# upb-lea/gym-electric-motor

Measured on AMD Instinct MI355X. Metric: env-steps/sec (batched PMSM, tau=1e-4), higher is better.
Workload: dtype f32; 1 GPU; Finite-CC-PMSM-v0 (Finite-B6C + dq transform), RK4, fp32, tau=1e-4, default constraint + auto-reset; 16384 envs/GPU x 1 GPU(s); one bench step = one fused launch of 1000 control steps, obs [K,N,S_out] rows + done bytes written for every control step; env_id=Finite-CC-PMSM-v0, envs_per_gpu=16384, solver=rk4, steps_per_launch=1000, parallelism=env-sharded x1, no data-path collective, world_size=1, oversubscribed=False

## Files before the change

### gym_electric_motor_amd/csrc/gemx_capi.hip

```cpp
#include <dlfcn.h>

#include <cstdarg>
#include <cstdio>
#include <cstdlib>
#include <cstring>
#include <mutex>
#include <new>
#include <set>
#include <string>

#include "gemx_common.hpp"

namespace gemx {

template <class R>
__device__ void reset_obs_row(int sys, const DevParams<R> &P, const double *y, double eps, int nd, int nout, double *o) {
    const double us = (double)P.u_sup, s3 = sqrt(3.0);
    for (int j = 0; j < nout; ++j) o[j] = 0.0;
    const double ua = -0.5 * us, ual = 2.0 / 3.0 * (ua - 0.5 * ua - 0.5 * ua), ube = 2.0 / 3.0 * (0.5 * s3 * ua - 0.5 * s3 * ua);
    if (eps > kPi) eps -= kTwoPi;
    if (sys == GEMX_SYS_SYNC || sys == GEMX_SYS_EESM) {
        const double c = cos(eps), s = sin(eps);
        const double al = c * y[1] - s * y[2], be = s * y[1] + c * y[2];
        o[0] = y[0];
// ... 593 lines not shown

    int ndev = 0;
    if (hipGetDeviceCount(&ndev) != hipSuccess || ndev <= 0) {
        delete h;
        return fail(GEMX_ERR_DEVICE, "no HIP device visible: the gemx stepper has no CPU fallback");
    }
    if (device < 0 || device >= ndev) { delete h; return fail(GEMX_ERR_ARG, "device %d out of range (0..%d)", device, ndev - 1); }
    gemx::DeviceGuard guard(device);
    {
        gemx_unit_launch_fn fn = nullptr;
        rc = load_unit(cfg->system_kind, h->conv_unit, cfg->dtype == GEMX_F64 ? 1 : 0, &fn);
        if (rc != GEMX_OK) { delete h; return rc; }
        h->unit_launch = (void *)fn;
    }
    {
        int cur = -1;
        if (hipGetDevice(&cur) != hipSuccess || cur != device) { delete h; return fail(GEMX_ERR_DEVICE, "hipSetDevice(%d) failed", device); }
        hipDeviceProp_t prop;
        if (hipGetDeviceProperties(&prop, device) == hipSuccess) {
            if (prop.multiProcessorCount > 0) h->n_cu = prop.multiProcessorCount;
            if (prop.sharedMemPerBlock >= 64 * 1024) h->lds_max = prop.sharedMemPerBlock;
            if (strncmp(prop.gcnArchName, "gfx950", 6) != 0 || prop.multiProcessorCount != 256) h->pace_gbps = 0.0;
        }
        for (const char *name : {"GEMX_STEPS_PER_BLOCK", "GEMX_PIPE", "GEMX_PIPE_SHAPE", "GEMX_STEP_KERNEL", "GEMX_DC_STREAM", "GEMX_DCS_EPW", "GEMX_LINMAP", "GEMX_PACE_GBPS", "GEMX_PACE_CAL"}) {
            const char *v = getenv(name);
            if (v == nullptr) continue;
            const size_t used = strlen(h->overrides);
            snprintf(h->overrides + used, sizeof(h->overrides) - used, "%s%s=%.16s", used ? " " : "", name, v);
        }
        const char *ev = getenv("GEMX_STEPS_PER_BLOCK");
        if (ev) h->steps_per_block = atoi(ev);
        ev = getenv("GEMX_PIPE");
        if (ev) h->use_pipe = atoi(ev);
        ev = getenv("GEMX_PIPE_SHAPE");
        if (ev) h->pipe_shape = atoi(ev);
        ev = getenv("GEMX_STEP_KERNEL");
        if (ev) h->use_step_kernel = atoi(ev);
        ev = getenv("GEMX_DC_STREAM");
        if (ev) h->use_dc_stream = atoi(ev);
        ev = getenv("GEMX_DCS_EPW");
        if (ev) h->dcs_epw = atoi(ev);
        ev = getenv("GEMX_PACE_GBPS");
        if (ev) h->pace_gbps = atof(ev);
        ev = getenv("GEMX_PACE_CAL");
        if (ev) h->pace_cal_on = atoi(ev);
        ev = getenv("GEMX_LINMAP");
        if (ev && atoi(ev) == 0) h->linmap_state = -1;

    }
    host_reset_obs(*h, m);

    const size_t es = (size_t)elem_size(h);
    auto cleanup = [&](int code) { gemx_destroy(h); return code; };
    h->extra_rows = (cfg->solver_flags & GEMX_SOLVER_ADAPTIVE) ? 3 : (cfg->supply_kind == GEMX_SUPPLY_RC ? 2 : 0);
    if (hipMalloc(&h->state, es * (h->nd + h->extra_rows) * (size_t)h->n) != hipSuccess) return cleanup(fail(GEMX_ERR_ALLOC, "hipMalloc(state) failed"));
    if (h->extra_rows && hipMemset((char *)h->state + es * (size_t)h->nd * (size_t)h->n, 0, es * (size_t)h->extra_rows * (size_t)h->n) != hipSuccess)
        return cleanup(fail(GEMX_ERR_DEVICE, "hipMemset failed"));
    if (h->has_angle && hipMalloc(&h->angle, (cfg->dtype == GEMX_F64 ? 8 : 4) * (size_t)h->n) != hipSuccess)
        return cleanup(fail(GEMX_ERR_ALLOC, "hipMalloc(angle) failed"));
    if (hipMalloc((void **)&h->sw, (size_t)h->n * h->sw_rows) != hipSuccess) return cleanup(fail(GEMX_ERR_ALLOC, "hipMalloc(sw) failed"));
    if (cfg->action_delay > 0) {
        const bool disc = c == GEMX_CONV_FINITE_B6 || c == GEMX_CONV_FINITE_4QC || c == GEMX_CONV_FINITE_2X4QC || c == GEMX_CONV_FINITE_B6_4QC ||
                          c == GEMX_CONV_FINITE_2XB6;
        h->ring_bytes = (size_t)cfg->action_delay * (size_t)h->n * (disc ? 1 : (size_t)h->nact_conv * es);
        if (hipMalloc(&h->ring, h->ring_bytes) != hipSuccess) return cleanup(fail(GEMX_ERR_ALLOC, "hipMalloc(delay ring) failed"));
    }
    if (cfg->init_kind != GEMX_INIT_CONST) {
        InitDev I;
        memset(&I, 0, sizeof(I));
        I.kind = cfg->init_kind;
// ... 366 lines not shown
    HIP_TRY(hipMemcpyAsync(out_dev, h->sw, (size_t)h->n * h->sw_rows, hipMemcpyDeviceToDevice, (hipStream_t)stream));
    return GEMX_OK;
}
int gemx_set_switch_state(gemx_handle *h, const uint8_t *in_dev, void *stream) {
    if (!h || !in_dev) return fail(GEMX_ERR_ARG, "null argument");
    gemx::DeviceGuard guard(h->device);
    HIP_TRY(hipMemcpyAsync(h->sw, in_dev, (size_t)h->n * h->sw_rows, hipMemcpyDeviceToDevice, (hipStream_t)stream));
    return GEMX_OK;
}
const char *gemx_last_launch(const gemx_handle *h) {
    if (!h) return "";
    const auto &l = h->ll;
    if (l.pipe == 3)
        snprintf(h->last_launch, sizeof(h->last_launch),
                 "gemx::dc_stream_kernel<sys=%d,conv=%d,solver=%d,f32,D=%d> grid=%lld x %d threads, lds=%zu B, K=%d", l.sys, l.conv, l.solver, l.d,
                 l.blocks, l.threads, l.lds, l.k);
    else if (l.pipe == 2)
        snprintf(h->last_launch, sizeof(h->last_launch), "gemx::step_kernel<sys=%d,conv=%d,load=%d,solver=%d,il=%d,%s> grid=%lld x %d threads, K=1", l.sys, l.conv,
                 l.load, l.solver, l.il, l.real_size == 4 ? "f32" : "f64", l.blocks, l.threads);
    else if (l.pipe) {
        snprintf(h->last_launch, sizeof(h->last_launch),
                 "gemx::advance_pipe_kernel<sys=%d,conv=%d,load=%d,solver=%d,il=%d,%s,D=%d> grid=%lld x %d threads, lds=%zu B, K=%d", l.sys,
                 l.conv, l.load, l.solver, l.il, l.real_size == 4 ? "f32" : "f64", l.d, l.blocks, l.threads, l.lds, l.k);
        if (l.pace != 0) {
            const size_t used = strlen(h->last_launch);
            snprintf(h->last_launch + used, sizeof(h->last_launch) - used, ", rate limit %u0 ns per block (%lld resident workgroups%s)", l.pace,
                     l.pace_res < l.blocks ? l.pace_res : l.blocks, l.pace_tail != 0 ? "; shorter in the last round" : "");
        }
        if (h->pace_cal_state != 0) {
            const size_t used = strlen(h->last_launch);
            snprintf(h->last_launch + used, sizeof(h->last_launch) - used, ", limiter %s at %.2f x the built-in target%s", h->pace_cal_state == 2 ? "calibrated" : "calibrating",
                     h->pace_scale_last, h->pace_scale_last == 0.0 ? " (unpaced)" : "");
        }
    } else
        snprintf(h->last_launch, sizeof(h->last_launch),
                 "gemx::advance_kernel<sys=%d,conv=%d,load=%d,solver=%d,il=%d,%s> grid=%lld x %d threads, lds=%zu B, K=%d, S=%d", l.sys, l.conv,
                 l.load, l.solver, l.il, l.real_size == 4 ? "f32" : "f64", l.blocks, l.threads, l.lds, l.k, l.s);
    if (h->overrides[0] != 0) {
        const size_t used = strlen(h->last_launch);
        snprintf(h->last_launch + used, sizeof(h->last_launch) - used, " overrides[%s]", h->overrides);
    }
    return h->last_launch;
}
int gemx_set_steps_per_block(gemx_handle *h, int32_t steps) {
    if (!h || steps < 0) return fail(GEMX_ERR_ARG, "invalid argument");
    h->steps_per_block = steps;
// ... 12 lines not shown
```

### gym_electric_motor_amd/csrc/gemx_common.hpp

```cpp
#pragma once
#include <hip/hip_runtime.h>

#include <cmath>
#include <cstdint>
#include <cstring>
#include <type_traits>

#include "gemx.h"

namespace gemx {

constexpr int BLOCK = 64;
constexpr double kTwoPi = 6.283185307179586476925286766559;
constexpr double kPi = 3.141592653589793238462643383279;

template <int SYS> struct SysTraits;
template <> struct SysTraits<GEMX_SYS_DC_PERMEX> { static constexpr int ND = 2, NOUT = 5, HAS_ANGLE = 0; };
template <> struct SysTraits<GEMX_SYS_SYNC>      { static constexpr int ND = 3, NOUT = 14, HAS_ANGLE = 1; };
template <> struct SysTraits<GEMX_SYS_SCIM>      { static constexpr int ND = 5, NOUT = 14, HAS_ANGLE = 1; };
template <> struct SysTraits<GEMX_SYS_DC_SERIES> { static constexpr int ND = 2, NOUT = 5, HAS_ANGLE = 0; };
template <> struct SysTraits<GEMX_SYS_DC_SHUNT>  { static constexpr int ND = 3, NOUT = 6, HAS_ANGLE = 0; };
template <> struct SysTraits<GEMX_SYS_DC_EXTEX>  { static constexpr int ND = 3, NOUT = 7, HAS_ANGLE = 0; };
template <> struct SysTraits<GEMX_SYS_EESM>      { static constexpr int ND = 4, NOUT = 16, HAS_ANGLE = 1; };
template <> struct SysTraits<GEMX_SYS_DFIM>      { static constexpr int ND = 5, NOUT = 24, HAS_ANGLE = 1; };
// ... 365 lines not shown
    unsigned char *ring;
    uint32_t *fifo_phase;
    uint32_t *err;
    const InitDev *rinit;
    uint32_t *rcnt;
    const RewardDev<R> *rw;
    const R *refs;
    R *reward;
    int64_t N;
    int32_t K, obs_every;
    int32_t S;
    int32_t D;
    int32_t coop;
    int32_t obs_vec;
    uint32_t pace_block_ticks;
    uint32_t pace_tail_ticks;
    uint32_t pace_tail_from;
    uint64_t act_seed;
    int64_t act_env_base;
    int32_t prep_phases;
    int32_t act_half;
    uint32_t act_step0;
    int32_t act_synth;
};

template <class R> __device__ __forceinline__ int fifo_phase_read(const KArgs<R> &a) {
    return a.P.delay > 0 ? (int)*a.fifo_phase : 0;
}
template <class R> __device__ __forceinline__ void fifo_phase_advance(const KArgs<R> &a, int phase, bool one_lane) {
    if (a.P.delay > 0 && one_lane) {
        const uint32_t ticket = atomicAdd(a.fifo_phase + 1, 1u);
        if (ticket == gridDim.x - 1) {
            a.fifo_phase[1] = 0u;
            a.fifo_phase[0] = (uint32_t)((phase + a.K) % a.P.delay);
        }
    }
}

constexpr int MAX_ACT_CHUNKS = 12;
constexpr int MAX_STEPS_PER_BLOCK = 32;
constexpr int PIPE_D = 12, PIPE_OUT_WAVES = 3;
constexpr int PIPE_D2 = 4, PIPE_OUT_WAVES2 = 2;
constexpr int PIPE_OUT_WAVES_RW = 6;
constexpr int PIPE_D3 = 2, PIPE_OUT_WAVES3 = 2;
constexpr int pipe_loader_waves(int) { return 1; }
constexpr int PIPE_ACT_BUFS = 2;
#ifndef GEMX_PIPE_AHEAD2
#define GEMX_PIPE_AHEAD2 0
#endif
constexpr int pipe_act_ahead(int D) { return (D <= 4 && GEMX_PIPE_AHEAD2) ? 2 : 1; }
constexpr int pipe_act_bufs(int D) { return pipe_act_ahead(D) + 1; }
constexpr int pipe_ref_bufs(int D) { return pipe_act_ahead(D) + 2; }
__host__ __device__ constexpr int pipe_queue_rows(int D, int delay, bool dq_processor, bool full) {
    return (D == PIPE_D && !full && dq_processor && delay > 0) ? D + delay : delay;
}
__host__ __device__ constexpr int act_chunks(int cpr) {
    return (MAX_STEPS_PER_BLOCK * cpr + BLOCK - 1) / BLOCK < MAX_ACT_CHUNKS ? (MAX_STEPS_PER_BLOCK * cpr + BLOCK - 1) / BLOCK : MAX_ACT_CHUNKS;
}

}

struct gemx_handle {
    gemx_config cfg;
    int64_t n;
    int device;
    int nd, nout, nact, has_angle;
// ... 14 lines not shown
    gemx::RewardHot<float> rh_f = {};
    gemx::RewardHot<double> rh_d = {};
    int rw_n_ref = -1;
    bool cur_half = false;
    bool cur_synth = false;
    uint64_t cur_seed = 0;
    uint32_t cur_step0 = 0;
    const void *cur_refs = nullptr;
    void *cur_reward = nullptr;
    void *ring = nullptr;
    size_t ring_bytes = 0;
    int nact_conv = 1;
    int conv_unit = 0;
    void *unit_launch = nullptr;
    unsigned long long steps_total = 0;
    uint32_t *fifo_phase = nullptr;
    uint32_t *err = nullptr;
    void *reset_obs_dev = nullptr;
    void *cw_dev = nullptr;
    double reset_obs[GEMX_MAX_OUT];
    int n_cu = 256;
    size_t lds_max = 160 * 1024;
    int steps_per_block = 0;
    struct LastLaunch { int pipe, sys, conv, load, solver, il, real_size, d, threads, k, s; long long blocks; size_t lds; unsigned pace, pace_tail; long long pace_res; int shape; };
    LastLaunch ll = {};
    mutable char last_launch[512] = "";
    char overrides[192] = "";
    double pace_gbps = -1.0;
    struct PaceCal {
        static constexpr int NC = 5, SAMPLES = 6, RING = 16;
        long long sig = -1;
        float center = 1.0f;
        int recenters = 0;
        static constexpr int MAX_RECENTER = 4;
        int next = 0;
        int chosen = -1;
        float best[NC] = {1e30f, 1e30f, 1e30f, 1e30f, 1e30f};
        int count[NC] = {0, 0, 0, 0, 0};
        int issued[NC] = {0, 0, 0, 0, 0};
        void *ev0[RING] = {}, *ev1[RING] = {};
        int ev_cand[RING];
        bool ev_init = false;
    } pcal;
    int pace_cal_on = 1;
    double pace_scale_last = 1.0;
    int pace_cal_state = 0;
    size_t pipe_occ_smem[8] = {0, 0, 0, 0, 0, 0, 0, 0};
    int pipe_occ[8] = {0, 0, 0, 0, 0, 0, 0, 0};
    int pipe_regs[8] = {0, 0, 0, 0, 0, 0, 0, 0};
// ... 45 lines not shown
```

### gym_electric_motor_amd/csrc/gemx_kernels.hpp

```cpp
#pragma once
#include <cstdio>

#include "gemx_common.hpp"

namespace gemx {

__device__ __forceinline__ float med3_r(float x, float lo, float hi) { return __builtin_amdgcn_fmed3f(x, lo, hi); }
__device__ __forceinline__ double med3_r(double x, double lo, double hi) { return fmin(fmax(x, lo), hi); }
template <class R> __device__ __forceinline__ R poly_load_ode(const DevParams<R> &P, R omega, R torque) {
    const R a = med3_r(P.lin_factor * omega, -P.la, P.la);
    const R tl = P.lc * (omega * fabs(omega)) + P.lb * omega + a;
    return (torque - tl) * P.inv_j;
}

template <int SYS, class R> struct Elec;

template <class R> struct Elec<GEMX_SYS_DC_PERMEX, R> {
    static constexpr int NM = 1;
    struct Pre { R b; };
    static __device__ __forceinline__ Pre prep(const DevParams<R> &P, R w, const R (&u)[MAX_U]) {
        const R bw = P.m[0] * w;
        return Pre{fma(P.m[2], u[0], bw)};
    }
    static __device__ __forceinline__ void f(const DevParams<R> &P, const Pre &p, const R (&x)[1], R (&dx)[1]) { dx[0] = p.b + P.m[1] * x[0]; }
// ... 814 lines not shown
    }
}
template <int SYS, int SOLVER, class R, bool LIN>
__device__ __forceinline__ void elec_apply(const DevParams<R> &P, R om, R (&x)[Elec<SYS, R>::NM], const R (&in)[Elec<SYS, R>::NM], const R *L) {
    using E = Elec<SYS, R>;
    constexpr int NM = E::NM;
    if (LIN) {
        R xn[NM];
#pragma unroll
        for (int r = 0; r < NM; ++r) {
            R acc = in[r];
#pragma unroll
            for (int c = 0; c < NM; ++c) acc += L[r * NM + c] * x[c];
            xn[r] = acc;
        }
#pragma unroll
        for (int r = 0; r < NM; ++r) x[r] = xn[r];
    } else {
        const R zu[MAX_U] = {R(0), R(0), R(0), R(0)};
        const typename E::Pre pre = E::set_b(E::prep(P, om, zu), in);
        auto rhs = [&](const R (&xx)[NM], R (&dx)[NM]) { E::f(P, pre, xx, dx); };
        rk_step<SOLVER, NM, R>(x, P.tau, rhs);
    }
}

template <bool IL, class R> __device__ __forceinline__ R cont_leg(const DevParams<R> &P, R duty, R i) {
    if (!IL) return duty;
    return clip01(duty - sgn(i) * P.il_ratio);
}
template <class R> __device__ __forceinline__ R fin_leg_u(uint32_t st, R i, R half_us) {
    const bool upper = (st == 1u) | ((st == 0u) & (i < R(0)));
    return upper ? half_us : -half_us;
}
constexpr uint32_t b6_subactions_of(uint32_t a) {
    return ((a & 4u) ? 1u : 2u) | (((a & 2u) ? 1u : 2u) << 2) | (((a & 1u) ? 1u : 2u) << 4);
}
__device__ __forceinline__ uint32_t b6_subactions(uint32_t a) { return b6_subactions_of(a); }
constexpr uint64_t b6_subaction_table() {
    uint64_t t = 0;
    for (uint32_t a = 0; a < 8; ++a) t |= (uint64_t)b6_subactions_of(a) << (6 * a);
    return t;
}
__device__ __forceinline__ uint32_t b6_subactions_packed(uint32_t a) {
    constexpr uint64_t T = b6_subaction_table();
    return (uint32_t)(T >> (6u * (a & 7u))) & 63u;
}
// ... 1399 lines not shown
    typedef volatile __attribute__((address_space(3))) uint32_t lds_u32_t;
    typedef volatile __attribute__((address_space(3))) u4_t lds_u4_t;
    constexpr int PREP_Q = prep_q<SYS>();
    lds_u32_t *prep = (lds_u32_t *)reinterpret_cast<uint32_t *>(vtab + ((ST::NVT > 0 && DISCRETE) ? ConvTraits<CONV>::NACTIONS * 8 : 0));
    lds_u32_t *prep_cnt = prep + (size_t)PREP_Q * BLOCK * 8;
    static_assert(ND + 1 <= 7, "a prepared draw is eight dwords: states, angle, tag");
#ifndef GEMX_PREP_DESC_COPY
#define GEMX_PREP_DESC_COPY 2
#endif
    InitDev *desc_lds = reinterpret_cast<InitDev *>(gemx_smem);
    if constexpr (FULL && RINIT) {
        desc_lds = reinterpret_cast<InitDev *>(reinterpret_cast<uint32_t *>(vtab + ((ST::NVT > 0 && DISCRETE) ? ConvTraits<CONV>::NACTIONS * 8 : 0)) +
                                              (size_t)(PREP_Q * 8 + 1) * BLOCK);
    }
    auto copy_desc_to_lds = [&]() {
        if constexpr (FULL && RINIT && GEMX_PREP_DESC_COPY == 2) {
            static_assert(sizeof(InitDev) % 4 == 0, "dword copy");
            const uint32_t *src = reinterpret_cast<const uint32_t *>(a.rinit);
            uint32_t *dst = reinterpret_cast<uint32_t *>(desc_lds);
            for (int i = tid; i < (int)(sizeof(InitDev) / 4); i += BLOCK) dst[i] = src[i];
        }
    };
    constexpr bool COMPACT_K = USE_TAB && SYS == GEMX_SYS_SYNC && linable<SYS, LOAD, SOLVER, IL, R>() && ST::NVT <= 5;
    auto steps_of = [&](int b) { return (K - b * D) < D ? (K - b * D) : D; };

    constexpr int ABYTES = DISCRETE ? 1 : NACT * (int)sizeof(R);
    constexpr int ROWB = BLOCK * ABYTES;
    constexpr int DP = ROWB == 64 ? (D + 3) / 4 * 4 : D;
    constexpr int U16 = ROWB / 16, NU16 = D * U16, NSTAGE = (NU16 + 63) / 64;
    auto stage_actions = [&](int b) {
        const int sb = steps_of(b);
        unsigned char *dst = actb + (size_t)(b % NBUF) * DP * ROWB;
        if (a.act_synth) {
            for (int s = 0; s < D; ++s) {
                const uint32_t t = a.act_step0 + (uint32_t)(b * D + (s < sb ? s : sb - 1));
                if constexpr (DISCRETE) {
                    dst[(size_t)s * ROWB + tid] = (unsigned char)synth_index(synth_u32(a.act_seed, a.act_env_base + envc, t, 0u), (uint32_t)ConvTraits<CONV>::NACTIONS);
                } else {
#pragma unroll
                    for (int i = 0; i < NACT; ++i) reinterpret_cast<R *>(dst + (size_t)s * ROWB)[tid * NACT + i] = (R)synth_unit(synth_u32(a.act_seed, a.act_env_base + envc, t, (uint32_t)i));
                }
            }
            return;
        }
        if constexpr (!DISCRETE && sizeof(R) == 4) {
            if (a.act_half) {
// ... 308 lines not shown
                        n_inline += 1u;
#endif
                    }
                    if (GEMX_PREP_DRAWS != 0) prep_cnt[tid] = rcount;
                    prefetch_draw();
                }
                sup[0] = rs ? P.u_sup : sup[0];
                sup[1] = rs ? R(0) : sup[1];
            }
            if constexpr (MODE == 2 || MODE == 3) since = rs ? 0u : (since < delay_u ? since + 1u : delay_u);
            if (FIFO && P.delay > 0) {
                if (rs) {
                    for (int d = 0; d < P.delay; ++d) {
#pragma unroll
                        for (int i = 0; i < NACTC; ++i) fifo[((size_t)d * BLOCK + tid) * NACTC + i] = P.dreset[i];
                    }
#pragma unroll
                    for (int i = 0; i < NACTC; ++i) pop[i] = P.dreset[i];
                }
            }
        };
        stage_actions(0);
        if (n_ref > 0) stage_refs(0);
        if (LW != 0 && DISCRETE) {
            __builtin_amdgcn_s_waitcnt(0x0F70);
            __syncthreads();
        }
#ifdef GEMX_TIMING
        unsigned long long tv = 0, tc = 0, tw = 0, tlong = 0, T0 = clock64(), W0 = wall_clock64(), t0, t0b, t1, t2;
#endif
        constexpr bool PIPE_PACED = !(D == PIPE_D && OW == PIPE_OUT_WAVES_RW);
        uint32_t pace = 0u;
        unsigned long long pace_t0 = 0ull;
        if constexpr (PIPE_PACED) {
            pace = blockIdx.x >= a.pace_tail_from ? a.pace_tail_ticks : a.pace_block_ticks;
            pace_t0 = pace != 0u ? wall_clock64() : 0ull;
        }
        for (int b = 0; b < nb; ++b) {
            if constexpr (PIPE_PACED) {
                if (pace != 0u) {
                    const unsigned long long due = pace_t0 + (unsigned long long)b * pace;
                    while (wall_clock64() < due) __builtin_amdgcn_s_sleep(4);
                }
            }
#ifdef GEMX_TIMING
            t0 = clock64();
// ... 61 lines not shown
#pragma unroll
                            for (int j = 0; j < ST::NVT; ++j) ec[j] = queued ? ec[j] : e0[j];
                            if constexpr (COMPACT_K) dc = queued ? dc : P.dreset_d;
                        }
                        one_step(Mode{}, ac, dc, hb + (size_t)s * BLOCK * NHT, ec);
                    }
                } else {
#pragma unroll 4
                    for (int s = 0; s < NS; ++s) {
                        dc = dn;
#pragma unroll
                        for (int i = 0; i < NACT; ++i) ac[i] = an[i];
                        rd(s + 1 < NS ? s + 1 : s, an, dn);
                        if constexpr (DEL) {
                            const bool queued = since >= delay_u;
                            dc = queued ? dc : P.dreset_d;
#pragma unroll
                            for (int i = 0; i < NACT; ++i) ac[i] = queued ? ac[i] : (i < NACTC ? P.dreset[i < NACTC ? i : 0] : R(0));
                        }
                        one_step(Mode{}, ac, dc, hb + (size_t)s * BLOCK * NHT, nullptr);
                    }
                }
            };
            bool compact_blk = false;
            using WholeBlock = std::integral_constant<int, D>;
            constexpr bool TAIL48 = D == PIPE_D && PIPE_D == 12 && SYS == GEMX_SYS_SYNC;
            if ((sb == D || (TAIL48 && (sb == 4 || sb == 8))) && P.delay == 0 && (!LINABLE || lin_ok) && !slow_path) {
                if (sb == D) run_block(std::false_type{}, WholeBlock{});
                else if constexpr (TAIL48) {
                    if (sb == 8) run_block(std::false_type{}, std::integral_constant<int, 8>{});
                    else run_block(std::false_type{}, std::integral_constant<int, 4>{});
                }
                compact_blk = COMPACT_K;
            } else if (CAN_DELAY && delayed) {
                compact_blk = COMPACT_K;
                if constexpr (CAN_DELAY) {
                    if (sb == D) {
                        run_block(std::true_type{}, WholeBlock{});
                    } else {
                        R ect[8] = {};
#pragma nounroll
                        for (int s = 0; s < sb; ++s) {
                            read_delayed(s, ac, dc);
                            const bool queued = since >= delay_u;
                            dc = queued ? dc : P.dreset_d;
#pragma unroll
                            for (int i = 0; i < NACT; ++i) ac[i] = queued ? ac[i] : (i < NACTC ? P.dreset[i < NACTC ? i : 0] : R(0));
                            if constexpr (USE_TAB) fetch_entry(dc, ect);
                            one_step(std::integral_constant<int, 2>{}, ac, dc, hb + (size_t)s * BLOCK * NHT, ect);
                        }
// ... 46 lines not shown
                            one_step(Mode3{}, ac, 0u, hb + (size_t)s * BLOCK * NHT, nullptr, qrow(s + P.delay), qrow(s + 1));
                        }
                    }
                    for (int j = 0; j < P.delay; ++j) {
                        R v[NACTC];
#pragma unroll
                        for (int i = 0; i < NACTC; ++i) v[i] = qrow(sb + j)[i];
#pragma unroll
                        for (int i = 0; i < NACTC; ++i) qrow(j)[i] = v[i];
                    }
                }
            } else {
                read_action(b, 0, an, dn);
#pragma nounroll
                for (int s = 0; s < sb; ++s) {
                    dc = dn;
#pragma unroll
                    for (int i = 0; i < NACT; ++i) ac[i] = an[i];
                    read_action(b, s + 1 < sb ? s + 1 : s, an, dn);
                    one_step(std::integral_constant<int, 1>{}, ac, dc, hb + (size_t)s * BLOCK * NHT, nullptr);
                }
            }
            if constexpr (COMPACT_K) {
                if (tid == 0) vtab[6 + (b & 1)] = compact_blk ? R(1) : R(0);
            }
#ifdef GEMX_TIMING
            t1 = clock64();
#endif
            __syncthreads();
#ifdef GEMX_TIMING
            t2 = clock64();
            tv += t0b - t0; tc += t1 - t0b; tw += t2 - t1;
            tlong += (t2 - t1) > 1000 ? 1 : 0;
            if (blockIdx.x == 0 && tid == 0 && b >= 100 && b < 148) {
                unsigned long long *tr = reinterpret_cast<unsigned long long *>(reinterpret_cast<char *>(a.err) + 64) + 64 + 0 * 96 + 2 * (b - 100);
                tr[0] = t1; tr[1] = t2;
            }
#endif
        }
#ifdef GEMX_TIMING
        if (tid == 0 && (blockIdx.x == 0 || blockIdx.x == 37)) {
            unsigned long long *dbg = reinterpret_cast<unsigned long long *>(reinterpret_cast<char *>(a.err) + 64) + (blockIdx.x ? 16 : 0);
            dbg[0] = tv; dbg[1] = tc; dbg[2] = tw; dbg[3] = clock64() - T0; dbg[4] = wall_clock64() - W0; dbg[5] = (unsigned long long)nb | (tlong << 32);
        }
        if (tid == 0 && blockIdx.x < 1024) {
            uint32_t hw, xcc;
            asm volatile("s_getreg_b32 %0, hwreg(HW_REG_HW_ID)" : "=s"(hw));
// ... 25 lines not shown
#endif
            }
            if (SOLVER == GEMX_SOLVER_DP5 && P.adaptive) a.state[(int64_t)(ND + 2) * N + env] = hcar;
            int phase_end = 0;
            if (P.delay > 0) phase_end = (ring_phase + K) % P.delay;
            for (int d = 0; d < P.delay; ++d) {
                int dst = d;
                bool keep = true;
                if (delayed_any) {
                    dst = phase_end + d;
                    dst = dst >= P.delay ? dst - P.delay : dst;
                    keep = (uint32_t)d + since >= delay_u;
                }
#pragma unroll
                for (int i = 0; i < NACTC; ++i) {
                    const int64_t gi = ((int64_t)dst * N + env) * NACTC + i;
                    const R v = keep ? fifo[((size_t)d * BLOCK + tid) * NACTC + i] : P.dreset[i];
                    if (DISCRETE) a.ring[gi] = (unsigned char)(uint32_t)v;
                    else reinterpret_cast<R *>(a.ring)[gi] = v;
                }
            }
        }
        if (bad_action) atomicOr(a.err, 1u);
        fifo_phase_advance(a, ring_phase, tid == 0);
    } else if (LW != 0 && wave == 1 + OW) {
#ifdef GEMX_TIMING
        unsigned long long tl = 0, tb = 0, tph[6] = {0, 0, 0, 0, 0, 0}, nph[6] = {0, 0, 0, 0, 0, 0};
#endif
        uint32_t bad = 0;
        uint32_t pq0[4] = {0u, 0u, 0u, 0u}, pq1[4] = {0u, 0u, 0u, 0u}, pp0[4] = {0u, 0u, 0u, 0u}, pp1[4] = {0u, 0u, 0u, 0u}, prep_c = 0u;
        uint32_t lq0[4] = {0u, 0u, 0u, 0u}, prep_lastw = 0u;
        bool prep_act = false;
        int prep_phase = 0;
        InitDev prep_desc;
        if constexpr (FULL && RINIT && GEMX_PREP_DRAWS != 0 && GEMX_PREP_DESC_COPY == 1) prep_desc = *a.rinit;
        copy_desc_to_lds();
        if (DISCRETE) __syncthreads();
        if (AHEAD == 2 && 1 < nb) {
            stage_actions(1);
            if (n_ref > 0) stage_refs(1);
        }
        for (int b = 0; b < nb; ++b) {
#ifdef GEMX_TIMING
            const unsigned long long l0 = clock64();
#endif
            const bool issued = b + AHEAD < nb;
            if (issued) {
                stage_actions(b + AHEAD);
                if (n_ref > 0) stage_refs(b + AHEAD);
            }
            if constexpr (FULL && RINIT && GEMX_PREP_DRAWS != 0) {
#pragma unroll 1
                for (int prep_rep = 0; prep_rep < a.prep_phases; ++prep_rep) {
#ifdef GEMX_TIMING
                    const unsigned long long pt0 = clock64();
                    const int pt_phase = prep_phase;
#endif
                    constexpr bool FLUX = SYS == GEMX_SYS_SCIM || SYS == GEMX_SYS_DFIM;
                    const InitDev *I = GEMX_PREP_DESC_COPY == 2 ? desc_lds : (GEMX_PREP_DESC_COPY == 1 ? &prep_desc : a.rinit);
// ... 69 lines not shown
#ifdef GEMX_TIMING
            const unsigned long long l1 = clock64();
#endif
            __syncthreads();
#ifdef GEMX_TIMING
            tl += l1 - l0; tb += clock64() - l1;
            if (blockIdx.x == 0 && tid == 0 && b >= 100 && b < 148) {
                unsigned long long *tr = reinterpret_cast<unsigned long long *>(reinterpret_cast<char *>(a.err) + 64) + 64 + 3 * 96 + 2 * (b - 100);
                tr[0] = l1; tr[1] = clock64();
            }
#endif
        }
        if (bad) atomicOr(a.err, 1u);
#ifdef GEMX_TIMING
        if (tid == 0 && (blockIdx.x == 0 || blockIdx.x == 37)) {
            unsigned long long *dbg = reinterpret_cast<unsigned long long *>(reinterpret_cast<char *>(a.err) + 64) + (blockIdx.x ? 16 : 0);
            dbg[12] = tl; dbg[13] = tb;
            if (blockIdx.x == 0) for (int i = 0; i < 6; ++i) { dbg[484 + i] = tph[i]; dbg[490 + i] = nph[i]; }
        }
#endif
    } else {
        const bool aos = P.obs_layout == GEMX_OBS_AOS;
        auto one_row = [&](auto compact_tag, const R (&row)[NHT], int rs) {
            constexpr bool COMPACT = decltype(compact_tag)::value;
            R y[ND], ho[NH], obs[NOUT];
            AngT ang = AngT(0);
            R dn;
            if constexpr (COMPACT) {
                uint32_t pk;
                memcpy(&pk, &row[2], sizeof(R));
                memcpy(&ang, &row[3], sizeof(R));
                const R *e = vtab + (size_t)(pk & 0xFFu) * 8;
                y[0] = P.init[0]; y[1] = row[0]; y[2] = row[1];
                ho[0] = row[4]; ho[1] = row[5]; ho[2] = e[2]; ho[3] = e[3]; ho[4] = e[4]; ho[5] = row[6]; ho[6] = row[7];
                dn = (pk & 0x100u) ? R(1) : R(0);
            } else {
#pragma unroll
                for (int j = 0; j < ND; ++j) y[j] = row[ST::row_slot(j)];
                if (HAS_ANGLE) {
                    const R bits = row[ST::row_slot(ND)];
                    memcpy(&ang, &bits, sizeof(R));
                }
#pragma unroll
                for (int j = 0; j < NH; ++j) ho[j] = row[ST::row_slot(ND + (HAS_ANGLE ? 1 : 0) + j)];
                dn = row[ST::row_slot(NDONE)];
            }
            ST::observe(P, y, ang, ho, obs);
            if constexpr (FULL) obs[NOUT - 1] = row[ST::row_slot(NDONE + 1)] * P.inv_lim[NOUT - 1];
            if (aos) {
#pragma unroll
                for (int j = 0; j < NOUT; ++j) ring[(rs * BLOCK + tid) * NOUT + j] = obs[j];
            } else {
#pragma unroll
                for (int j = 0; j < NOUT; ++j) ring[(rs * NOUT + j) * BLOCK + tid] = obs[j];
            }
            donebuf[rs * BLOCK + tid] = dn != R(0) ? 1 : 0;
        };
        auto load_row = [&](auto compact_tag, const R *src, R (&row)[NHT]) {
#pragma unroll
            for (int j = 0; j < (decltype(compact_tag)::value ? 8 : NHT); ++j) row[j] = src[j];
        };
        static_assert(D % OW == 0, "rows per output wave");
        constexpr int RPW = D / OW;
        const int ow = wave - 1;
        const int r0 = ow * RPW;
        auto rows_of = [&](int pb) {
            const int sb = steps_of(pb);
            return sb - r0 < RPW ? (sb - r0 < 0 ? 0 : sb - r0) : RPW;
        };

#ifdef GEMX_TIMING
        unsigned long long tflush = 0;
#endif
        auto process = [&](int pb) {
            const int nr = rows_of(pb);
            if (nr <= 0) return;
            const R *hb = hand + (size_t)(pb & 1) * D * BLOCK * NHT + (size_t)r0 * BLOCK * NHT + (size_t)tid * NHT;
            R rows[2][NHT];
            auto convert_rows = [&](auto compact_tag) {
                load_row(compact_tag, hb, rows[0]);
                if (nr == RPW) {
#pragma unroll
                    for (int s = 0; s < RPW; ++s) {
                        if (s + 1 < RPW) load_row(compact_tag, hb + (size_t)(s + 1) * BLOCK * NHT, rows[(s + 1) & 1]);
                        one_row(compact_tag, rows[s & 1], r0 + s);
                    }
                } else {
#pragma unroll
                    for (int s = 0; s < RPW; ++s) {
                        if (s < nr) {
                            if (s + 1 < nr) load_row(compact_tag, hb + (size_t)(s + 1) * BLOCK * NHT, rows[(s + 1) & 1]);
                            one_row(compact_tag, rows[s & 1], r0 + s);
                        }
                    }
                }
            };
            if constexpr (COMPACT_K) {
                if (__builtin_amdgcn_readfirstlane(__builtin_bit_cast(int, vtab[6 + (pb & 1)])) != 0) convert_rows(std::true_type{});
                else convert_rows(std::false_type{});
            } else {
                convert_rows(std::false_type{});
            }
#ifdef GEMX_TIMING
            const unsigned long long f0 = clock64();
#endif
            if (a.rw != nullptr) {
                RewardRegs<R> WR;
                WR.load(a.rh);
                R rv[RPW][GEMX_MAX_REF];
                const R *rb = refb + ((size_t)(pb % NRBUF) * D + r0) * BLOCK * n_ref + (size_t)tid * n_ref;
                auto fetch_refs = [&](int nrr) {
#pragma unroll
                    for (int s = 0; s < RPW; ++s) {
#pragma unroll
                        for (int j = 0; j < GEMX_MAX_REF; ++j) {
                            const R v = rb[(size_t)(s < nrr ? s : 0) * BLOCK * n_ref + (j < n_ref ? j : 0)];
                            rv[s][j] = (s < nrr && j < n_ref) ? v : R(0);
                        }
                    }
                };
                if (nr == RPW) {
                    fetch_refs(RPW);
                    reward_apply<NOUT, RPW, R>(a, WR, ring, donebuf, pb * D + r0, r0, RPW, tid, env, valid, rv);
                } else {
                    fetch_refs(nr);
                    reward_apply<NOUT, RPW, R>(a, WR, ring, donebuf, pb * D + r0, r0, nr, tid, env, valid, rv);
                }
            }
            if (aos && nr == RPW && fast_io) flush_rows_pipe<NOUT, RPW, R>(a, ring + (size_t)r0 * BLOCK * NOUT, donebuf + (size_t)r0 * BLOCK, pb * D + r0, tid, blk0);
            else flush_rings<NOUT, R>(a, ring + (size_t)r0 * BLOCK * NOUT, donebuf + (size_t)r0 * BLOCK, pb * D + r0, nr, tid, blk0, rows_n, full_wg,
                                      valid, env);
#ifdef GEMX_TIMING
            tflush += clock64() - f0;
#endif
        };
#ifdef GEMX_TIMING
        unsigned long long tp = 0, tq = 0, pmax = 0, pg2 = 0, pg3 = 0;
#endif
        if (LW != 0 && DISCRETE) __syncthreads();
        for (int b = 0; b < nb; ++b) {
#ifdef GEMX_TIMING
            const unsigned long long q0 = clock64();
#endif
            if (b >= 1) process(b - 1);
#ifdef GEMX_TIMING
            const unsigned long long q1 = clock64();
#endif
            __syncthreads();
#ifdef GEMX_TIMING
            tp += q1 - q0; tq += clock64() - q1;
            pmax = (q1 - q0) > pmax ? (q1 - q0) : pmax; pg2 += (q1 - q0) > 2000; pg3 += (q1 - q0) > 3000;
            if (blockIdx.x == 0 && tid == 0 && b >= 100 && b < 148) {
                unsigned long long *tr = reinterpret_cast<unsigned long long *>(reinterpret_cast<char *>(a.err) + 64) + 64 + (wave < 3 ? wave : 2) * 96 + 2 * (b - 100);
                tr[0] = q1; tr[1] = clock64();
            }
#endif
        }
        process(nb - 1);
#ifdef GEMX_TIMING
        if (tid == 0 && (blockIdx.x == 0 || blockIdx.x == 37)) {
            unsigned long long *dbg = reinterpret_cast<unsigned long long *>(reinterpret_cast<char *>(a.err) + 64) + (blockIdx.x ? 16 : 0);
// ... 535 lines not shown
        S = (int)((lds_max - 1024) / per_cu / per_step);
        if (S > MAX_STEPS_PER_BLOCK) S = MAX_STEPS_PER_BLOCK;
    }
    const int cpr = BLOCK * abytes / 16;
    const int s_regs = act_chunks(cpr) * BLOCK / cpr;
    if (S > s_regs) S = s_regs;
    const int s_lds = (int)((lds_max - 256) / per_step);
    if (S > s_lds) S = s_lds;
    if (S > K) S = K;
    if (S < 1) S = 1;
    return S;
}

template <int SYS, int CONV, int LOAD, int SOLVER, bool IL, class R>
int launch_advance_t(gemx_handle *h, const void *actions, int K, void *obs, uint8_t *done, int obs_every, hipStream_t st) {
    constexpr int ABYTES = ConvTraits<CONV>::DISCRETE ? 1 : ConvTraits<CONV>::NACT * (int)sizeof(R);
    KArgs<R> a;
    a.P = params_of<R>(h);
    a.state = (R *)h->state;
    a.angle = (typename Angle<R>::T *)h->angle;
    a.sw = h->sw;
    a.actions = (const unsigned char *)actions;
    a.act_synth = h->cur_synth ? 1 : 0;
    a.act_seed = h->cur_seed;
    a.act_env_base = h->cfg.env_base;
    a.act_half = h->cur_half ? 1 : 0;
#ifdef GEMX_PREP_PHASES
    a.prep_phases = GEMX_PREP_PHASES;
#else
    a.prep_phases = ((SYS == GEMX_SYS_SCIM || SYS == GEMX_SYS_DFIM) && (h->n + BLOCK - 1) / BLOCK <= (int64_t)h->n_cu) ? 2 : 1;
#endif
    a.act_step0 = h->cur_step0;
    a.obs = (R *)obs;
    a.done = done;
    a.ring = (unsigned char *)h->ring;
    const int delay = h->cfg.action_delay;
    a.fifo_phase = h->fifo_phase;
    a.err = h->err;
    if (h->linmap_state == 0) {
        if constexpr (linable<SYS, LOAD, SOLVER, IL, R>()) {
            hipStreamCaptureStatus capturing = hipStreamCaptureStatusNone;
            (void)hipStreamIsCapturing(st, &capturing);
            const bool omega_drawn = h->cfg.init_kind != GEMX_INIT_CONST && h->cfg.init_lo[0] < h->cfg.init_hi[0];
            if (omega_drawn || (h->cfg.solver_flags & GEMX_SOLVER_ADAPTIVE) || h->cfg.solver_nsteps != 1) {
                h->linmap_state = -1;
            } else if (capturing == hipStreamCaptureStatusNone) {
// ... 240 lines not shown
                        }
                    }
                    const int use = pc.chosen >= 0 ? pc.chosen : (cal_slot >= 0 ? cal_cand : 0);
                    target *= CAL_SCALE[use] * pc.center;
                    pace_scale_used = CAL_SCALE[use] * pc.center;
                }
                int64_t res = shape >= 4 ? resident(D, OW, shape) : resident(D, OW);
                if (res > 4 * (int64_t)h->n_cu && blocks <= res && blocks > res - (int64_t)h->n_cu) res -= (int64_t)h->n_cu;
                pace_res = res;
                if (target > 0.0 && (blocks > (int64_t)h->n_cu || h->pace_gbps > 0.0 || long_one) && K >= 64 && shape != 3 && shape < 5) {
                    const double wg_step_bytes = (double)BLOCK * ((h->cur_synth ? 0 : abytes_eff) + h->nout * sizeof(R) + 1 + (h->cur_reward != nullptr ? (h->rw_n_ref + 1) * sizeof(R) : 0));
                    auto ticks_for = [&](double active) {
                        const double t = wg_step_bytes * active / target * D / 10.0;
                        return t < 1.0 ? 1u : (t > 4.0e9 ? 0u : (uint32_t)(t + 0.5));
                    };
                    const int64_t full = blocks / res, tail = blocks - full * res;
                    a.pace_block_ticks = ticks_for((double)(blocks < res ? blocks : res));
                    if (full >= 1 && tail > 0) {
                        a.pace_tail_from = (uint32_t)(full * res);
                        a.pace_tail_ticks = ticks_for((double)(tail < (int64_t)h->n_cu ? (int64_t)h->n_cu : tail));
                    }
                }
            }
            const size_t psmem = smem_of(D);
            auto pkern = pipe_kernel_of<SYS, CONV, LOAD, SOLVER, IL, R>(shape);
            if (pkern == nullptr) return fail(GEMX_ERR_ARG, "internal: pipelined shape %d is not built for this solver", shape);
            if (!(h->pipe_attr_set & (1u << shape))) {
                GEMX_HIP_TRY(hipFuncSetAttribute((const void *)pkern, hipFuncAttributeMaxDynamicSharedMemorySize, (int)h->lds_max));
                h->pipe_attr_set |= 1u << shape;
            }
            const int threads = (1 + OW + pipe_loader_waves(D)) * BLOCK;
            if (cal_slot >= 0) (void)hipEventRecord((hipEvent_t)h->pcal.ev0[cal_slot], st);
            hipLaunchKernelGGL(pkern, dim3((unsigned)blocks), dim3(threads), psmem, st, a);
            if (cal_slot >= 0 && hipEventRecord((hipEvent_t)h->pcal.ev1[cal_slot], st) != hipSuccess) { h->pcal.ev_cand[cal_slot] = -1; (void)hipGetLastError(); }
            GEMX_HIP_TRY(hipGetLastError());
            h->pace_scale_last = pace_scale_used;
            h->pace_cal_state = h->pcal.chosen >= 0 ? 2 : (cal_slot >= 0 ? 1 : 0);
            h->ll = {1, SYS, CONV, LOAD, SOLVER, (int)IL, (int)sizeof(R), D, threads, K, D, (long long)blocks, psmem, a.pace_block_ticks, a.pace_tail_ticks, (long long)pace_res};
            h->ll.shape = shape;
            return GEMX_OK;
        }
    }
    if (h->cur_half)
        return fail(GEMX_ERR_ARG, "gemx_rollout_half needs the pipelined kernel: fp32, K >= 2, a continuous converter (and no random initial states together with solver sub-steps / a custom constraint set)");
    if (h->cur_synth)
        return fail(GEMX_ERR_ARG, "gemx_rollout_synthetic needs the pipelined kernel: fp32, K >= 2 (and no random initial states together with solver sub-steps / a custom constraint set)");
    if (K == 1 && h->cur_reward == nullptr && h->use_step_kernel != 0) {
        if (h->step_fn == nullptr && !h->step_fn_failed) {
            hipFunction_t f = nullptr;
            if (hipGetFuncBySymbol(&f, (const void *)step_kernel<SYS, CONV, LOAD, SOLVER, IL, R>) == hipSuccess && f != nullptr) h->step_fn = (void *)f;
            else { h->step_fn_failed = true; (void)hipGetLastError(); }
        }
        if (h->step_fn != nullptr) {
            size_t sz = sizeof(a);
            void *cfg[] = {HIP_LAUNCH_PARAM_BUFFER_POINTER, (void *)&a, HIP_LAUNCH_PARAM_BUFFER_SIZE, &sz, HIP_LAUNCH_PARAM_END};
            GEMX_HIP_TRY(hipModuleLaunchKernel((hipFunction_t)h->step_fn, (unsigned)blocks, 1, 1, BLOCK, 1, 1, 0, st, nullptr, cfg));
        } else {
            hipLaunchKernelGGL((step_kernel<SYS, CONV, LOAD, SOLVER, IL, R>), dim3((unsigned)blocks), dim3(BLOCK), 0, st, a);
            GEMX_HIP_TRY(hipGetLastError());
        }
        h->ll = {2, SYS, CONV, LOAD, SOLVER, (int)IL, (int)sizeof(R), 0, BLOCK, K, 1, (long long)blocks, 0};
        return GEMX_OK;
// ... 47 lines not shown
```

Before: 110.7 billion env-steps/s.

## Add LDS table of precomputed per-angle input vectors for linear PMSM step

```diff
diff --git a/gym_electric_motor_amd/csrc/gemx_capi.hip b/gym_electric_motor_amd/csrc/gemx_capi.hip
--- a/gym_electric_motor_amd/csrc/gemx_capi.hip
+++ b/gym_electric_motor_amd/csrc/gemx_capi.hip
@@ -639,7 +639,7 @@
             if (prop.sharedMemPerBlock >= 64 * 1024) h->lds_max = prop.sharedMemPerBlock;
             if (strncmp(prop.gcnArchName, "gfx950", 6) != 0 || prop.multiProcessorCount != 256) h->pace_gbps = 0.0;
         }
-        for (const char *name : {"GEMX_STEPS_PER_BLOCK", "GEMX_PIPE", "GEMX_PIPE_SHAPE", "GEMX_STEP_KERNEL", "GEMX_DC_STREAM", "GEMX_DCS_EPW", "GEMX_LINMAP", "GEMX_PACE_GBPS", "GEMX_PACE_CAL"}) {
+        for (const char *name : {"GEMX_STEPS_PER_BLOCK", "GEMX_PIPE", "GEMX_PIPE_SHAPE", "GEMX_STEP_KERNEL", "GEMX_DC_STREAM", "GEMX_DCS_EPW", "GEMX_LINMAP", "GEMX_PACE_GBPS", "GEMX_PACE_CAL", "GEMX_TABLE_STEP"}) {
             const char *v = getenv(name);
             if (v == nullptr) continue;
             const size_t used = strlen(h->overrides);
@@ -663,6 +663,8 @@
         if (ev) h->pace_cal_on = atoi(ev);
         ev = getenv("GEMX_LINMAP");
         if (ev && atoi(ev) == 0) h->linmap_state = -1;
+        ev = getenv("GEMX_TABLE_STEP");
+        if (ev) h->table_step = atoi(ev);
 
     }
     host_reset_obs(*h, m);
@@ -1075,6 +1077,10 @@
         snprintf(h->last_launch, sizeof(h->last_launch),
                  "gemx::advance_pipe_kernel<sys=%d,conv=%d,load=%d,solver=%d,il=%d,%s,D=%d> grid=%lld x %d threads, lds=%zu B, K=%d", l.sys,
                  l.conv, l.load, l.solver, l.il, l.real_size == 4 ? "f32" : "f64", l.d, l.blocks, l.threads, l.lds, l.k);
+        if (l.tab != 0) {
+            const size_t used = strlen(h->last_launch);
+            snprintf(h->last_launch + used, sizeof(h->last_launch) - used, ", table_step rows=%d", l.tab);
+        }
         if (l.pace != 0) {
             const size_t used = strlen(h->last_launch);
             snprintf(h->last_launch + used, sizeof(h->last_launch) - used, ", rate limit %u0 ns per block (%lld resident workgroups%s)", l.pace,
diff --git a/gym_electric_motor_amd/csrc/gemx_common.hpp b/gym_electric_motor_amd/csrc/gemx_common.hpp
--- a/gym_electric_motor_amd/csrc/gemx_common.hpp
+++ b/gym_electric_motor_amd/csrc/gemx_common.hpp
@@ -411,6 +411,7 @@
     int32_t act_half;
     uint32_t act_step0;
     int32_t act_synth;
+    int32_t tab_n;
 };
 
 template <class R> __device__ __forceinline__ int fifo_phase_read(const KArgs<R> &a) {
@@ -431,6 +432,7 @@
 constexpr int PIPE_D = 12, PIPE_OUT_WAVES = 3;
 constexpr int PIPE_D2 = 4, PIPE_OUT_WAVES2 = 2;
 constexpr int PIPE_OUT_WAVES_RW = 6;
+constexpr int PIPE_TAB_ROWS = 512;
 constexpr int PIPE_D3 = 2, PIPE_OUT_WAVES3 = 2;
 constexpr int pipe_loader_waves(int) { return 1; }
 constexpr int PIPE_ACT_BUFS = 2;
@@ -491,9 +493,10 @@
     int n_cu = 256;
     size_t lds_max = 160 * 1024;
     int steps_per_block = 0;
-    struct LastLaunch { int pipe, sys, conv, load, solver, il, real_size, d, threads, k, s; long long blocks; size_t lds; unsigned pace, pace_tail; long long pace_res; int shape; };
+    struct LastLaunch { int pipe, sys, conv, load, solver, il, real_size, d, threads, k, s; long long blocks; size_t lds; unsigned pace, pace_tail; long long pace_res; int shape; int tab; };
     LastLaunch ll = {};
     mutable char last_launch[512] = "";
+    int table_step = 1;
     char overrides[192] = "";
     double pace_gbps = -1.0;
     struct PaceCal {
diff --git a/gym_electric_motor_amd/csrc/gemx_kernels.hpp b/gym_electric_motor_amd/csrc/gemx_kernels.hpp
--- a/gym_electric_motor_amd/csrc/gemx_kernels.hpp
+++ b/gym_electric_motor_amd/csrc/gemx_kernels.hpp
@@ -860,6 +860,29 @@
         auto rhs = [&](const R (&xx)[NM], R (&dx)[NM]) { E::f(P, pre, xx, dx); };
         rk_step<SOLVER, NM, R>(x, P.tau, rhs);
     }
+}
+
+template <int SYS, class R> __device__ __forceinline__ void lin_step_g(const R *L, const R (&g)[Elec<SYS, R>::NG], R (&y)[SysTraits<SYS>::ND]) {
+    static_assert(SYS == GEMX_SYS_SYNC, "x-first form of the whole-step map");
+    constexpr int NM = Elec<SYS, R>::NM, NG = Elec<SYS, R>::NG;
+    R x[NM], xn[NM];
+#pragma unroll
+    for (int i = 0; i < NM; ++i) x[i] = y[1 + i];
+#pragma unroll
+    for (int r = 0; r < NM; ++r) {
+        R acc = fma(L[NM * NM + r * NG], g[0], x[r]);
+#pragma unroll
+        for (int i = 1; i < NG; ++i) acc += L[NM * NM + r * NG + i] * g[i];
+#pragma unroll
+        for (int c = 0; c < NM; ++c) acc += L[r * NM + c] * x[c];
+        xn[r] = acc;
+    }
+#pragma unroll
+    for (int i = 0; i < NM; ++i) y[1 + i] = xn[i];
+}
+template <class R> __device__ __forceinline__ void sync_udq(R s, R c, R ual, R ube, R &ud, R &uq) {
+    ud = c * ual + s * ube;
+    uq = -s * ual + c * ube;
 }
 
 template <bool IL, class R> __device__ __forceinline__ R cont_leg(const DevParams<R> &P, R duty, R i) {
@@ -2305,6 +2328,29 @@
         }
     };
     constexpr bool COMPACT_K = USE_TAB && SYS == GEMX_SYS_SYNC && linable<SYS, LOAD, SOLVER, IL, R>() && ST::NVT <= 5;
+    constexpr bool TABSTEP = COMPACT_K && D == PIPE_D && OW == PIPE_OUT_WAVES_RW && sizeof(R) == 4;
+    [[maybe_unused]] R *gtab = vtab + ((ST::NVT > 0 && DISCRETE) ? ConvTraits<CONV>::NACTIONS * 8 : 0);
+    [[maybe_unused]] uint32_t tab_delta = 0u;
+    [[maybe_unused]] const AngT tab_ang0 = Angle<R>::from_bits(P.init_angle_rep);
+    if constexpr (TABSTEP) tab_delta = (uint32_t)Angle<R>::increment(P.pole * P.init[0] * P.tau);
+    auto build_gtab = [&]() {
+        if constexpr (TABSTEP) {
+            if (a.tab_n > 0) {
+                const uint32_t act = threadIdx.x & 7u;
+                static_assert(!TABSTEP || ConvTraits<CONV>::NACTIONS == 8, "table rows of eight actions");
+                R e[8];
+                ST::action_entry(P, act, e);
+                for (uint32_t n = threadIdx.x >> 3; n < (uint32_t)a.tab_n; n += blockDim.x >> 3) {
+                    R s, c, u[MAX_U] = {R(0), R(0), R(0), R(0)}, g[2];
+                    Angle<R>::sincos(Angle<R>::add(tab_ang0, (typename Angle<R>::Inc)(n * tab_delta)), s, c);
+                    sync_udq(s, c, e[0], e[1], u[0], u[1]);
+                    Elec<SYS, R>::get_b(Elec<SYS, R>::prep(P, P.init[0], u), g);
+                    gtab[(n * 8u + act) * 2u] = g[0];
+                    gtab[(n * 8u + act) * 2u + 1u] = g[1];
+                }
+            }
+        }
+    };
     auto steps_of = [&](int b) { return (K - b * D) < D ? (K - b * D) : D; };
 
     constexpr int ABYTES = DISCRETE ? 1 : NACT * (int)sizeof(R);
@@ -2659,6 +2705,18 @@
         };
         stage_actions(0);
         if (n_ref > 0) stage_refs(0);
+        build_gtab();
+        [[maybe_unused]] uint32_t tab_nn = 0u, tab_t = 0u, tab_inv = 1u, n_tabblk = 0u;
+        [[maybe_unused]] bool tab_have = false;
+        if constexpr (TABSTEP) {
+            if (tab_delta != 0u) {
+                tab_t = (uint32_t)__builtin_ctz(tab_delta);
+                const uint32_t m = tab_delta >> tab_t;
+                tab_inv = m;
+#pragma unroll
+                for (int i = 0; i < 4; ++i) tab_inv *= 2u - m * tab_inv;
+            }
+        }
         if (LW != 0 && DISCRETE) {
             __builtin_amdgcn_s_waitcnt(0x0F70);
             __syncthreads();
@@ -2766,10 +2824,59 @@
                     }
                 }
             };
+            [[maybe_unused]] auto run_block_tab = [&]() {
+                if constexpr (TABSTEP) {
+                    typedef R r2_t __attribute__((ext_vector_type(2)));
+                    typedef R r4_t __attribute__((ext_vector_type(4)));
+                    const r2_t *gt = reinterpret_cast<const r2_t *>(gtab);
+                    const R nh[NH] = {};
+                    uint32_t n = tab_nn, dnn = 0;
+                    const uint32_t ninc = tab_delta != 0u ? 1u : 0u;
+                    read_action(b, 0, an, dn);
+                    read_action(b, 1, an, dnn);
+                    r2_t gv = gt[n * 8u + (dn & AMASK)];
+#pragma unroll 4
+                    for (int s = 0; s < D; ++s) {
+                        dc = dn & AMASK;
+                        dn = dnn;
+                        read_action(b, s + 2 < D ? s + 2 : D - 1, an, dnn);
+                        const R g[2] = {gv.x, gv.y};
+                        lin_step_g<SYS, R>(linc, g, y);
+                        const R viol = ST::state_violation(P, y, nh);
+                        const bool done = viol > thr_done, rs = viol > thr_reset;
+                        const uint32_t pk = (done ? 0x100u : 0u) | dc;
+                        r4_t rowv;
+                        rowv.x = y[1]; rowv.y = y[2]; rowv.z = __builtin_bit_cast(R, pk); rowv.w = __builtin_bit_cast(R, n);
+                        *reinterpret_cast<r4_t *>(hb + (size_t)s * BLOCK * NHT) = rowv;
+#pragma unroll
+                        for (int j = 1; j < ND; ++j) y[j] = rs ? init_v[j] : y[j];
+                        n = rs ? 0u : n + ninc;
+                        gv = gt[n * 8u + (dn & AMASK)];
+                    }
+                    tab_nn = n;
+                    ang = Angle<R>::add(tab_ang0, (typename Angle<R>::Inc)(n * tab_delta));
+                }
+            };
+            bool tab_blk = false;
+            if constexpr (TABSTEP) {
+                if (a.tab_n > 0 && sb == D && P.delay == 0 && lin_ok) {
+                    bool ok = true;
+                    if (!tab_have) {
+                        const uint32_t diff = (uint32_t)ang - (uint32_t)tab_ang0;
+                        tab_nn = tab_delta != 0u ? (((diff >> tab_t) * tab_inv) & (0xFFFFFFFFu >> tab_t)) : 0u;
+                        ok = tab_nn * tab_delta == diff;
+                    }
+                    tab_blk = __all(ok && tab_nn + (uint32_t)D < (uint32_t)a.tab_n);
+                }
+                tab_have = tab_blk;
+                n_tabblk += tab_blk ? 1u : 0u;
+            }
             bool compact_blk = false;
             using WholeBlock = std::integral_constant<int, D>;
             constexpr bool TAIL48 = D == PIPE_D && PIPE_D == 12 && SYS == GEMX_SYS_SYNC;
-            if ((sb == D || (TAIL48 && (sb == 4 || sb == 8))) && P.delay == 0 && (!LINABLE || lin_ok) && !slow_path) {
+            if (tab_blk) {
+                run_block_tab();
+            } else if ((sb == D || (TAIL48 && (sb == 4 || sb == 8))) && P.delay == 0 && (!LINABLE || lin_ok) && !slow_path) {
                 if (sb == D) run_block(std::false_type{}, WholeBlock{});
                 else if constexpr (TAIL48) {
                     if (sb == 8) run_block(std::false_type{}, std::integral_constant<int, 8>{});
@@ -2862,7 +2969,7 @@
                 }
             }
             if constexpr (COMPACT_K) {
-                if (tid == 0) vtab[6 + (b & 1)] = compact_blk ? R(1) : R(0);
+                if (tid == 0) vtab[6 + (b & 1)] = tab_blk ? R(2) : (compact_blk ? R(1) : R(0));
             }
 #ifdef GEMX_TIMING
             t1 = clock64();
@@ -2934,6 +3041,13 @@
             }
         }
         if (bad_action) atomicOr(a.err, 1u);
+        if constexpr (TABSTEP) {
+            if (a.tab_n > 0 && tid == 0) {
+                unsigned long long *dbgc = reinterpret_cast<unsigned long long *>(reinterpret_cast<char *>(a.err) + 64);
+                atomicAdd(&dbgc[502], (unsigned long long)n_tabblk);
+                atomicAdd(&dbgc[503], (unsigned long long)((uint32_t)nb - n_tabblk));
+            }
+        }
         fifo_phase_advance(a, ring_phase, tid == 0);
     } else if (LW != 0 && wave == 1 + OW) {
 #ifdef GEMX_TIMING
@@ -2947,6 +3061,7 @@
         InitDev prep_desc;
         if constexpr (FULL && RINIT && GEMX_PREP_DRAWS != 0 && GEMX_PREP_DESC_COPY == 1) prep_desc = *a.rinit;
         copy_desc_to_lds();
+        build_gtab();
         if (DISCRETE) __syncthreads();
         if (AHEAD == 2 && 1 < nb) {
             stage_actions(1);
@@ -3062,11 +3177,21 @@
     } else {
         const bool aos = P.obs_layout == GEMX_OBS_AOS;
         auto one_row = [&](auto compact_tag, const R (&row)[NHT], int rs) {
-            constexpr bool COMPACT = decltype(compact_tag)::value;
+            constexpr bool COMPACT = decltype(compact_tag)::value == 1, TABROW = decltype(compact_tag)::value == 2;
             R y[ND], ho[NH], obs[NOUT];
             AngT ang = AngT(0);
             R dn;
-            if constexpr (COMPACT) {
+            if constexpr (TABROW) {
+                const uint32_t pk = __builtin_bit_cast(uint32_t, row[2]), n = __builtin_bit_cast(uint32_t, row[3]);
+                const R *e = vtab + (size_t)(pk & 0xFFu) * 8;
+                const AngT a0 = Angle<R>::add(tab_ang0, (typename Angle<R>::Inc)(n * tab_delta));
+                Angle<R>::sincos(a0, ho[0], ho[1]);
+                ang = Angle<R>::add(a0, (typename Angle<R>::Inc)tab_delta);
+                y[0] = P.init[0]; y[1] = row[0]; y[2] = row[1];
+                ho[2] = e[2]; ho[3] = e[3]; ho[4] = e[4];
+                sync_udq(ho[0], ho[1], e[0], e[1], ho[5], ho[6]);
+                dn = (pk & 0x100u) ? R(1) : R(0);
+            } else if constexpr (COMPACT) {
                 uint32_t pk;
                 memcpy(&pk, &row[2], sizeof(R));
                 memcpy(&ang, &row[3], sizeof(R));
@@ -3098,7 +3223,7 @@
         };
         auto load_row = [&](auto compact_tag, const R *src, R (&row)[NHT]) {
 #pragma unroll
-            for (int j = 0; j < (decltype(compact_tag)::value ? 8 : NHT); ++j) row[j] = src[j];
+            for (int j = 0; j < (decltype(compact_tag)::value == 2 ? 4 : (decltype(compact_tag)::value == 1 ? 8 : NHT)); ++j) row[j] = src[j];
         };
         static_assert(D % OW == 0, "rows per output wave");
         constexpr int RPW = D / OW;
@@ -3136,10 +3261,13 @@
                 }
             };
             if constexpr (COMPACT_K) {
-                if (__builtin_amdgcn_readfirstlane(__builtin_bit_cast(int, vtab[6 + (pb & 1)])) != 0) convert_rows(std::true_type{});
-                else convert_rows(std::false_type{});
+                const int fmt = __builtin_amdgcn_readfirstlane(__builtin_bit_cast(int, vtab[6 + (pb & 1)]));
+                if (TABSTEP && fmt == __builtin_bit_cast(int, 2.0f)) {
+                    if constexpr (TABSTEP) convert_rows(std::integral_constant<int, 2>{});
+                } else if (fmt != 0) convert_rows(std::integral_constant<int, 1>{});
+                else convert_rows(std::integral_constant<int, 0>{});
             } else {
-                convert_rows(std::false_type{});
+                convert_rows(std::integral_constant<int, 0>{});
             }
 #ifdef GEMX_TIMING
             const unsigned long long f0 = clock64();
@@ -3177,6 +3305,7 @@
 #ifdef GEMX_TIMING
         unsigned long long tp = 0, tq = 0, pmax = 0, pg2 = 0, pg3 = 0;
 #endif
+        build_gtab();
         if (LW != 0 && DISCRETE) __syncthreads();
         for (int b = 0; b < nb; ++b) {
 #ifdef GEMX_TIMING
@@ -3758,6 +3887,7 @@
     a.sw = h->sw;
     a.actions = (const unsigned char *)actions;
     a.act_synth = h->cur_synth ? 1 : 0;
+    a.tab_n = 0;
     a.act_seed = h->cur_seed;
     a.act_env_base = h->cfg.env_base;
     a.act_half = h->cur_half ? 1 : 0;
@@ -4044,7 +4174,12 @@
                     }
                 }
             }
-            const size_t psmem = smem_of(D);
+            size_t psmem = smem_of(D);
+            if (shape == 3 && compact_l && h->table_step != 0 && delay == 0 && h->cur_reward == nullptr && fast_step &&
+                psmem + (size_t)PIPE_TAB_ROWS * 8 * 2 * sizeof(R) <= h->lds_max) {
+                a.tab_n = PIPE_TAB_ROWS;
+                psmem += (size_t)PIPE_TAB_ROWS * 8 * 2 * sizeof(R);
+            }
             auto pkern = pipe_kernel_of<SYS, CONV, LOAD, SOLVER, IL, R>(shape);
             if (pkern == nullptr) return fail(GEMX_ERR_ARG, "internal: pipelined shape %d is not built for this solver", shape);
             if (!(h->pipe_attr_set & (1u << shape))) {
@@ -4060,6 +4195,7 @@
             h->pace_cal_state = h->pcal.chosen >= 0 ? 2 : (cal_slot >= 0 ? 1 : 0);
             h->ll = {1, SYS, CONV, LOAD, SOLVER, (int)IL, (int)sizeof(R), D, threads, K, D, (long long)blocks, psmem, a.pace_block_ticks, a.pace_tail_ticks, (long long)pace_res};
             h->ll.shape = shape;
+            h->ll.tab = a.tab_n;
             return GEMX_OK;
         }
     }
```

Result: slower. 91.16 billion env-steps/s (-17.6%).
